# weiquan/salt

Measured on AMD Instinct MI355X. Metric: Mreads/s aligned (100 bp SE, GRCh38+snp144) at 1/2/4/8 MI355X vs CPU ref, higher is better.
Workload: dtype u32; 1 GPU; GRCh38-scale synthetic (SURVEY 8d config 3 = BASELINE configs[2]): 3100000000 bp genome in 24 contigs, 14800000 SNPs, k=21, 1000000 x 100 bp SE reads per GPU per step, 8 distinct resident batches rotated, inputs and results resident in HBM; read_len=100, distinct_batches=8, options=default (-s 50 -m 1000, overlap = k), streams_per_gpu=4

## Files before the change

### salt_amd/csrc/salt_align.hip

```cpp
#include <type_traits>
#include "salt_device.h"
#include "salt_kernels.h"

namespace salt {

#define WSYNC() do { __builtin_amdgcn_fence(__ATOMIC_ACQ_REL, "wavefront"); __builtin_amdgcn_wave_barrier(); \
                     __builtin_amdgcn_fence(__ATOMIC_ACQ_REL, "wavefront"); } while (0)

static constexpr int MAXL = SALT_MAX_READ_LEN;
static constexpr int SLOTS = SALT_MAX_SEED_SLOTS;
static constexpr int MAXLOC = SALT_MAX_LOCATE;
static constexpr int LVK = 31;
static_assert(offsetof(salt_result_t, strand) == 4 && offsetof(salt_result_t, mapq) == 7 && offsetof(salt_result_t, b0) == 8 &&
              offsetof(salt_result_t, b1) == 12 && offsetof(salt_result_t, seq_start) == 16 && offsetof(salt_result_t, seq_end) == 18 &&
              offsetof(salt_result_t, n_hits) == 20 && offsetof(salt_result_t, n_cigar) == 22 && offsetof(salt_result_t, skipped) == 23 &&
              offsetof(salt_result_t, hits) == 24 && sizeof(salt_hit_t) == 8, "salt_result_t header layout");
static constexpr int NHIT = 6;
__device__ __forceinline__ uint32_t mapq_quot(uint32_t x, uint32_t b0)
{
    const uint32_t v = 255u * x;
    return b0 == 1u ? v : b0 == 2u ? v / 2u : b0 == 3u ? v / 3u : v / b0;
}
static constexpr uint32_t INF = 255;

// ... 446 lines not shown
            n_lkt += __shfl_down(n_lkt, o); n_occ_c += __shfl_down(n_occ_c, o); n_occ_r += __shfl_down(n_occ_r, o);
        }
        if (lane_id() == 0) {
            atomicAdd(ctr + SALT_CTR_LKT, n_lkt & 1023u); atomicAdd(ctr + SALT_CTR_OCC_C, n_occ_c); atomicAdd(ctr + SALT_CTR_OCC_R, n_occ_r);
            atomicAdd(ctr + SALT_CTR_D_WLKT, n_lkt & 1023u); atomicAdd(ctr + SALT_CTR_D_COCC_SEED, n_occ_c); atomicAdd(ctr + SALT_CTR_D_ROCC_SEED, n_occ_r);
            atomicAdd(ctr + SALT_CTR_D_SA_SEED, (n_lkt >> 10) & 2047u); atomicAdd(ctr + SALT_CTR_D_TEXT_SEED, n_lkt >> 21);
        }
    }
}

__global__ void __launch_bounds__(256) __attribute__((amdgpu_waves_per_eu(4, 4)))
k_seed_walk(IndexView ix, SeedParams sp, const uint32_t *__restrict__ tb, uint4 *__restrict__ sai_c, uint4 *__restrict__ sai_r,
            const uint4 *__restrict__ wq, const uint32_t *__restrict__ wq_cnt, uint32_t wq_seg_cap, uint32_t r_first, unsigned long long *__restrict__ ctr)
{
    const uint32_t seg = blockIdx.x & (WQ_SEG - 1u);
    const uint32_t wv = (blockIdx.x / WQ_SEG) * 4u + (uint32_t)__builtin_amdgcn_readfirstlane((int)(threadIdx.x >> 6)), nw = (gridDim.x / WQ_SEG) * 4u;
    const uint64_t lt = (1ull << lane_id()) - 1ull;
    const uint32_t la = r_first ? 0u : 1u, lb = la ^ 1u;
    const uint32_t na = wq_cnt[(la * WQ_SEG + seg) * WQ_STRIDE], nb = wq_cnt[(lb * WQ_SEG + seg) * WQ_STRIDE];
    const uint32_t a0 = (uint32_t)((uint64_t)na * wv / nw), a1 = (uint32_t)((uint64_t)na * (wv + 1u) / nw);
    const uint32_t b0 = (uint32_t)((uint64_t)nb * wv / nw), b1 = (uint32_t)((uint64_t)nb * (wv + 1u) / nw);
    const uint4 *qa = wq + (((size_t)la * WQ_SEG + seg) * wq_seg_cap + a0) * WQ_REC, *qb = wq + (((size_t)lb * WQ_SEG + seg) * wq_seg_cap + b0) * WQ_REC;
    const uint32_t tot_a = a1 - a0, tot = tot_a + (b1 - b0);
    const int i_top = (int)((uint32_t)sp.l_seed - ix.r_lkt_len) - 1;
    uint32_t n_aux = 0, n_sa = 0, n_text = 0, n_occ_c = 0, n_occ_r = 0;
    Walk w; w.ph = WK_IDLE; w.k = w.l = w.ext = w.p0 = 0; w.i = 0;
    SeedCtx c = seed_ctx_geom(sp, tb, 0, ix.r_lkt_len);
    uint32_t item = 0, cur = 0;
    bool is_r = false;
    const uint4 *qp = qa;
    for (;;) {
        const uint64_t idle = __ballot(w.ph == WK_IDLE);
        if (cur >= tot && idle == ~0ull) break;
        if (cur < tot) {
            const uint32_t t = cur + (uint32_t)__popcll(idle & lt);
            if (w.ph == WK_IDLE && t < tot) {
                const bool in_a = t < tot_a;
                qp = in_a ? qa + (size_t)t * WQ_REC : qb + (size_t)(t - tot_a) * WQ_REC; is_r = (in_a ? la : lb) == 0u; w.ph = WK_REC;
            }
            const uint32_t nx = cur + (uint32_t)__popcll(idle);
            cur = nx < tot ? nx : tot;
        }
        WalkReq q = walk_req_none();
        if (w.ph == WK_REC) { q.pa = qp; q.na = WQ_REC; }
        else if (w.ph != WK_IDLE) q = is_r ? seed_walk_issue<true>(ix, sp, c, w) : seed_walk_issue<false>(ix, sp, c, w);
        const WalkLoads ld = walk_fetch(q);
        bool done = false;
        uint4 row = make_uint4(1, 0, 0, 0);
        if (w.ph == WK_REC) {
            item = ld.a[0].x;
            c = seed_ctx_geom(sp, tb, item, ix.r_lkt_len);
            c.w0 = ld.a[1].x; c.w1 = ld.a[1].y; c.w2 = ld.a[1].z; c.n0 = ld.a[0].w; c.n1 = ld.a[1].w;
            done = is_r ? seed_walk_begin<true>(sp, c, ld.a[0].y, ld.a[0].z, i_top, w, row) : seed_walk_begin<false>(sp, c, ld.a[0].y, ld.a[0].z, i_top, w, row);
        } else if (w.ph != WK_IDLE) {
            done = is_r ? seed_walk_finish<true>(ix, sp, c, w, ld, row, n_occ_r, n_aux) : seed_walk_finish<false>(ix, sp, c, w, ld, row, n_occ_c, n_aux);
        }
        if (done && row.x <= row.y) { if (is_r) { row.w = sai_r_pack(sp.epoch, row.w); sai_r[item] = row; } else sai_c[item] = row; }
        n_sa += (n_aux >> 10) & 2047u; n_text += n_aux >> 21; n_aux = 0;
    }
    if (ctr) {
        for (int o = 32; o > 0; o >>= 1) { n_sa += __shfl_down(n_sa, o); n_text += __shfl_down(n_text, o); n_occ_c += __shfl_down(n_occ_c, o); n_occ_r += __shfl_down(n_occ_r, o); }
        if (lane_id() == 0) {
            atomicAdd(ctr + SALT_CTR_OCC_C, n_occ_c); atomicAdd(ctr + SALT_CTR_OCC_R, n_occ_r);
            atomicAdd(ctr + SALT_CTR_D_COCC_SEED, n_occ_c); atomicAdd(ctr + SALT_CTR_D_ROCC_SEED, n_occ_r);
            atomicAdd(ctr + SALT_CTR_D_SA_SEED, n_sa); atomicAdd(ctr + SALT_CTR_D_TEXT_SEED, n_text);
        }
    }
}

template <int NS> struct SaiListsT { uint32_t sp[2][NS], ep[2][NS], off[2][NS]; };
struct SaiLists { uint32_t *sp[2], *ep[2], *off[2]; };
template <int NS> __device__ __forceinline__ SaiLists sai_ref(SaiListsT<NS> &a) { return SaiLists{ { a.sp[0], a.sp[1] }, { a.ep[0], a.ep[1] }, { a.off[0], a.off[1] } }; }
struct LvTables { short L[LVK][64]; char A[LVK][64]; };
static constexpr int LLV_K = 12;
static constexpr int LLV_TW = 22;
static constexpr int LLV_N = 64;
static constexpr int LLV_WIN = 4;
static constexpr int LLV_TS = LLV_TW + 2;
static constexpr int LLV_PW = LLV_TW;
static_assert(((8 * (LLV_TW - 1) - LLV_WIN + LLV_K) >> 3) + 2 <= LLV_TS, "text words of the longest window at the widest bound");
static_assert(((8 * (LLV_TW - 1) - LLV_WIN) >> 3) + 2 <= LLV_PW, "pattern words of the longest read");
struct LaneLv { uint32_t T[LLV_TS * LLV_N]; uint32_t P[LLV_PW]; };
struct LvBytes { uint8_t T[MAXL + 4 + 64]; uint8_t P[MAXL + 64]; };
template <int NS, bool LLV>
struct WaveLdsT {
    static constexpr bool HAS_LLV = LLV;
    static constexpr int N_SLOTS = NS;
    uint32_t pm[2][MAXL / 8];
    union U { SaiListsT<NS> sai; typename std::conditional<LLV, LaneLv, uint32_t>::type llv; LvBytes lvb; } u;
    uint8_t  cand_e[MAXLOC];
    uint32_t loci[MAXLOC];
    uint32_t hit_pos[2][NHIT];
    uint8_t  hit_nd[2][NHIT], hit_gap[2][NHIT];
    uint16_t cig[SALT_MAX_CIGAR_OPS];
    int      n_cig;
    alignas(8) uint8_t cargs[128];
};
typedef WaveLdsT<SLOTS, true> WaveLds;
typedef WaveLdsT<32, false> WaveLdsSmall;
typedef WaveLdsT<1, false> WaveLdsCigar;

struct Sai { uint32_t sp, ep, off; };
__device__ __forceinline__ Sai sai_get(const SaiLists &s, int w, int i) { return Sai{ s.sp[w][i], s.ep[w][i], s.off[w][i] }; }
__device__ __forceinline__ void sai_set(SaiLists &s, int w, int i, Sai v) { s.sp[w][i] = v.sp; s.ep[w][i] = v.ep; s.off[w][i] = v.off; }
__device__ __forceinline__ bool sai_ltv(Sai a, Sai b) { return a.ep - a.sp < b.ep - b.sp; }
__device__ __forceinline__ bool sai_lt(const SaiLists &s, int w, int i, int j) { return sai_ltv(sai_get(s, w, i), sai_get(s, w, j)); }
__device__ __forceinline__ void sai_swap(SaiLists &s, int w, int i, int j) { Sai a = sai_get(s, w, i), b = sai_get(s, w, j); sai_set(s, w, i, b); sai_set(s, w, j, a); }

__device__ void sai_insertsort(SaiLists &s, int w, int lo, int hi)
{
    for (int i = lo + 1; i < hi; ++i)
        for (int j = i; j > lo && sai_lt(s, w, j, j - 1); --j) sai_swap(s, w, j, j - 1);
}

__device__ void sai_combsort(SaiLists &s, int w, int base, int n)
{
    const double shrink = 1.2473309501039786540366528676643;
    int gap = n; bool do_swap;
    do {
        if (gap > 2) { gap = (int)(gap / shrink); if (gap == 9 || gap == 10) gap = 11; }
        do_swap = false;
        for (int i = 0; i < n - gap; ++i)
            if (sai_lt(s, w, base + i + gap, base + i)) { sai_swap(s, w, base + i, base + i + gap); do_swap = true; }
    } while (do_swap || gap > 2);
    if (gap != 1) sai_insertsort(s, w, base, base + n);
}

__device__ __attribute__((noinline)) void sai_introsort(SaiLists &s, int w, int n)
{
    if (n < 1) return;
    if (n == 2) { if (sai_lt(s, w, 1, 0)) sai_swap(s, w, 0, 1); return; }
    int d; for (d = 2; (1 << d) < n; ++d) { }
    d <<= 1;
    int st_l[24], st_r[24], st_d[24], top = 0;
    int lo = 0, hi = n - 1;
    for (;;) {
        if (lo < hi) {
            if (--d == 0) { sai_combsort(s, w, lo, hi - lo + 1); hi = lo; continue; }
            int i = lo, j = hi, k = i + ((j - i) >> 1) + 1;
            if (sai_lt(s, w, k, i)) { if (sai_lt(s, w, k, j)) k = j; }
            else k = sai_lt(s, w, j, i) ? i : j;
            Sai rp = sai_get(s, w, k);
            if (k != hi) sai_swap(s, w, k, hi);
            for (;;) {
                do ++i; while (sai_ltv(sai_get(s, w, i), rp));
                do --j; while (i <= j && sai_ltv(rp, sai_get(s, w, j)));
                if (j <= i) break;
                sai_swap(s, w, i, j);
            }
            sai_swap(s, w, i, hi);
            if (i - lo > hi - i) {
                if (i - lo > 16 && top < 24) { st_l[top] = lo; st_r[top] = i - 1; st_d[top] = d; ++top; }
                lo = hi - i > 16 ? i + 1 : hi;
            } else {
                if (hi - i > 16 && top < 24) { st_l[top] = i + 1; st_r[top] = hi; st_d[top] = d; ++top; }
                hi = i - lo > 16 ? i - 1 : lo;
            }
        } else {
            if (top == 0) { sai_insertsort(s, w, 0, n); return; }
            --top; lo = st_l[top]; hi = st_r[top]; d = st_d[top];
        }
    }
}

__device__ void sort_loci(uint32_t *a, uint32_t n)
{
    if (n < 2) return;
    uint32_t P = 2; while (P < n) P <<= 1;
    for (uint32_t i = n + lane_id(); i < P; i += 64) a[i] = 0xFFFFFFFFu;
    WSYNC();
    for (uint32_t k = 2; k <= P; k <<= 1) {
        for (uint32_t j = k >> 1; j > 0; j >>= 1) {
// ... 353 lines not shown
__device__ __forceinline__ void verify_quads_2(const uint32_t *__restrict__ ref, uint32_t ref_len, const uint32_t *pm0, const uint32_t *pm1, uint32_t L,
                                               const uint32_t *c0, uint32_t n0, const uint32_t *c1, uint32_t n1, uint8_t *o0, uint8_t *o1)
{
    constexpr uint32_t CPW = (uint32_t)GW / LN;
    const uint32_t lane = LaneGroup<GW>::lane(), sub = lane & (uint32_t)(LN - 1), q = lane / (uint32_t)LN;
    const uint32_t nw = (L + 7) >> 3, n = n0 + n1;
    const uint32_t nvalid = L > 32u * sub ? (L - 32u * sub < 32u ? L - 32u * sub : 32u) : 0u;
    const bool behind = LN == 8 && GW == 32 && !(4u * sub < nw + 1u);
    uint32_t pa[4], pb[4];
#pragma unroll
    for (int t = 0; t < 4; ++t) { const bool in = (4 * sub + t) < nw; pa[t] = in ? pm0[4 * sub + t] : 0u; pb[t] = in ? pm1[4 * sub + t] : 0u; }
    for (uint32_t b = 0; b < n; b += 4u * CPW) {
        uint32_t pos[4]; u32x4_a4 x[4]; bool act[4], rev[4];
#pragma unroll
        for (int g = 0; g < 4; ++g) {
            if (b + CPW * g >= n) break;
            const uint32_t c = b + CPW * g + q;
            act[g] = c < n; rev[g] = c >= n0;
            pos[g] = act[g] ? (rev[g] ? c1[c - n0] : c0[c]) : 0u;
            if (pos[g] >= ref_len) pos[g] = 0xFFFFFFFFu;
            if (behind) x[g] = u32x4_a4{ 0u, 0u, 0u, 0u };
            else x[g] = *reinterpret_cast<const u32x4_a4 *>(ref + ((pos[g] == 0xFFFFFFFFu ? 0u : pos[g]) >> 3) + 4 * sub);
        }
#pragma unroll
        for (int g = 0; g < 4; ++g) {
            if (b + CPW * g >= n) break;
            const uint32_t pw[4] = { rev[g] ? pb[0] : pa[0], rev[g] ? pb[1] : pa[1], rev[g] ? pb[2] : pa[2], rev[g] ? pb[3] : pa[3] };
            const uint32_t mism = quad_mismatch<LN>(x[g], pos[g], pw, nvalid);
            if (act[g] && sub == 0) {
                const uint32_t c = b + CPW * g + q;
                const uint8_t v = (uint8_t)((mism > 3 || pos[g] == 0xFFFFFFFFu) ? INF : mism);
                if (rev[g]) o1[c - n0] = v; else o0[c] = v;
            }
        }
    }
}

__device__ __attribute__((noinline)) int lv_wave(const uint8_t *T, int tlen, const uint8_t *P, int plen, int k, LvTables *tab, int &d_fin)
{
    const int lane = (int)lane_id();
    const int d = lane - 31;
    const int ad = d < 0 ? -d : d;
    int Lprev = -2;
    const int end0 = plen < tlen ? plen : tlen;
    if (d == 0) { int i = 0; while (i < end0 && (P[i] & T[i]) != 0) ++i; Lprev = i; }
    const int r0 = __shfl(Lprev, 31);
    if (tab) tab->L[0][lane] = (short)Lprev;
    d_fin = 0;
    if (r0 == end0) return plen > end0 ? plen - end0 : 0;
    if (k > LVK - 1) k = LVK - 1;
    for (int e = 1; e <= k; ++e) {
        int left = __shfl_up(Lprev, 1), right = __shfl_down(Lprev, 1);
        if (lane == 0) left = -2;
        if (lane == 63) right = -2;
        const bool active = ad <= e && ad <= LVK - 1;
        int best = Lprev + 1; char act = 'X';
        if (left > best) { best = left; act = 'D'; }
        if (right + 1 > best) { best = right + 1; act = 'I'; }
        int cur = -2;
        if (active) {
            if (P[best] == T[d + best]) {
                int end = plen < tlen - d ? plen : tlen - d;
                if (best >= end) best = end;
                else { int i = best; while (i < end && (P[i] & T[d + i]) != 0) ++i; best = i; }
            }
            cur = best;
        }
        if (tab) { tab->L[e][lane] = (short)cur; tab->A[e][lane] = act; }
        uint64_t reach = __ballot(active && cur == plen);
        if (reach) {
            if (tab) {
                int rank = d == 0 ? 0 : (d < 0 ? 2 * ad - 1 : 2 * ad);
                int my = (active && cur == plen) ? rank : 1000;
                for (int o = 32; o > 0; o >>= 1) { int t = __shfl_xor(my, o); my = t < my ? t : my; }
                d_fin = my == 0 ? 0 : ((my & 1) ? -((my + 1) >> 1) : (my >> 1));
            }
            return e;
        }
        Lprev = cur;
    }
    return -1;
}

__device__ __attribute__((noinline)) uint32_t lv_lanes(LaneLv &s, const uint32_t *pm, int plen, int tlen, int k, bool active)
{
    constexpr int LLV_W = 2 * LLV_K + 1;
    const int lane = (int)lane_id() & (LLV_N - 1);
    const lds_u32 T = as_lds(s.T) + lane, P = as_lds(pm);
    auto fetch = [&](int i, int t, uint32_t &p, uint32_t &x) {
        const lds_u32 pp = P + (i >> 3), tt = T + (t >> 3) * LLV_N;
        const uint32_t p0 = pp[0], p1 = pp[1], t0 = tt[0], t1 = tt[LLV_N];
        p = __funnelshift_r(p0, p1, 4u * (uint32_t)(i & 7));
        x = __funnelshift_r(t0, t1, 4u * (uint32_t)(t & 7));
    };
    auto run_of = [](uint32_t p, uint32_t x) -> int {
        const uint32_t y = p & x;
        const uint32_t z = ~(((y & 0x77777777u) + 0x77777777u) | y) & 0x88888888u;
        return z ? __builtin_ctz(z) >> 2 : 8;
    };
    auto reach = [&](int d, int best, bool gated) -> int {
        uint32_t p, x;
        fetch(best, d + best, p, x);
        const int end = plen < tlen - d ? plen : tlen - d;
        const bool open = !gated || ((p ^ x) & 15u) == 0;
        int run = run_of(p, x), i = best + run;
        if (open && run == 8) while (i < end) { fetch(i, d + i, p, x); run = run_of(p, x); i += run; if (run < 8) break; }
        i = i < end ? i : end;
        return open ? i : best;
    };
    int row[LLV_W];
#pragma unroll
    for (int j = 0; j < LLV_W; ++j) row[j] = -2;
    const int end0 = plen < tlen ? plen : tlen;
    uint32_t result = 255;
    bool done = !active;
    if (active) {
        const int i = reach(0, 0, false);
        row[LLV_K] = i;
        if (i == end0) { result = (uint32_t)(plen > end0 ? plen - end0 : 0); done = true; }
    }
    for (int e = 1; e <= k; ++e) {
        if (__ballot(!done) == 0) break;
        int carry = -2;
#pragma unroll
        for (int d = -LLV_K; d <= LLV_K; ++d) {
            if ((d < 0 ? -d : d) > e) continue;
            const int mid = row[d + LLV_K], right = d < LLV_K ? row[d + LLV_K + 1] : -2;
            int best = mid + 1;
            if (carry > best) best = carry;
            if (right + 1 > best) best = right + 1;
            carry = mid;
            if (!done) {
                best = reach(d, best, true);
                if (best == plen) { result = (uint32_t)e; done = true; }
                else row[d + LLV_K] = best;
            }
        }
    }
    return result;
}

template <int VMAX, bool GAPF>
__device__ __forceinline__ void rule_unsorted(const uint32_t *pos, const uint8_t *val, const uint32_t n, const uint32_t L, const uint32_t ref_len,
                                              uint32_t &bound, bool &any, uint32_t &best_pos, uint32_t &best_v,
                                              uint32_t &n_hits, uint32_t &a0, uint32_t *hit_pos, uint8_t *hit_nd)
{
    const uint32_t lane = lane_id();
    const uint32_t NONE = 0xFFFFFFFFu;
    auto in_range = [&](uint32_t p) -> bool { return GAPF ? !(p + L + 4 >= ref_len) : p < ref_len; };
    uint32_t mp[VMAX + 1];
#pragma unroll
    for (int t = 0; t <= VMAX; ++t) mp[t] = NONE;
    uint32_t my_p = 0, my_v = NONE, n_p = 0;
    for (uint32_t b = 0; b < n; b += 64) {
        const uint32_t i = b + lane;
        uint32_t p = 0, v = NONE;
        if (i < n) { p = pos[i]; v = val[i]; }
        const bool in = i < n && v <= bound && in_range(p);
        if (in) {
#pragma unroll
            for (int t = 0; t <= VMAX; ++t) if (v == (uint32_t)t && p < mp[t]) mp[t] = p;
        }
        uint64_t m = __ballot(in);
        if (m && n_p <= 64u) {
            if (n_p + (uint32_t)__popcll(m) > 64u) n_p = 65u;
            else
                while (m) {
                    const int l = __ffsll((long long)m) - 1;
                    const uint32_t pl = (uint32_t)__builtin_amdgcn_readlane((int)p, l), vl = (uint32_t)__builtin_amdgcn_readlane((int)v, l);
                    if (lane == n_p) { my_p = pl; my_v = vl; }
                    ++n_p; m &= m - 1;
                }
        }
    }
#pragma unroll
    for (int t = 0; t <= VMAX; ++t)
        for (int o = 32; o > 0; o >>= 1) { const uint32_t x = (uint32_t)__shfl_xor((int)mp[t], o); mp[t] = x < mp[t] ? x : mp[t]; }
    uint32_t before[VMAX + 1];
    before[0] = NONE;
#pragma unroll
    for (int t = 1; t <= VMAX; ++t) before[t] = mp[t - 1] < before[t - 1] ? mp[t - 1] : before[t - 1];
    any = false; n_hits = 0;
#pragma unroll
    for (int t = VMAX; t >= 0; --t) if (mp[t] != NONE) { any = true; best_v = (uint32_t)t; best_pos = mp[t]; }
    if (!any) return;
    unsigned long long last = 0;
    const bool in_lanes = n_p <= 64u;
    unsigned long long my_key = ~0ull;
    if (in_lanes && lane < n_p) {
        uint32_t lim = NONE;
#pragma unroll
        for (int t = 1; t <= VMAX; ++t) if (my_v == (uint32_t)t) lim = before[t];
        if (my_p < lim) my_key = ((unsigned long long)my_p << 8) | my_v;
    }
    for (uint32_t h = 0; h < (uint32_t)NHIT; ++h) {
        unsigned long long cur = ~0ull;
        if (in_lanes) { if (h == 0 || my_key > last) cur = my_key; }
        else
        for (uint32_t b = 0; b < n; b += 64) {
            const uint32_t i = b + lane;
            if (i < n) {
                const uint32_t p = pos[i], v = val[i];
                if (v <= bound && in_range(p)) {
                    uint32_t lim = NONE;
#pragma unroll
                    for (int t = 1; t <= VMAX; ++t) if (v == (uint32_t)t) lim = before[t];
                    const unsigned long long key = ((unsigned long long)p << 8) | v;
                    if (p < lim && (h == 0 || key > last) && key < cur) cur = key;
                }
            }
        }
        for (int o = 32; o > 0; o >>= 1) {
            const unsigned long long x = ((unsigned long long)(uint32_t)__shfl_xor((int)(cur >> 32), o) << 32) | (uint32_t)__shfl_xor((int)(uint32_t)cur, o);
            cur = x < cur ? x : cur;
        }
        if (cur == ~0ull) break;
        if (lane == 0) { hit_pos[h] = (uint32_t)(cur >> 8); hit_nd[h] = (uint8_t)(cur & 255u); }
        if (h == 0) a0 = (uint32_t)(cur & 255u);
        last = cur; ++n_hits;
    }
    bound = best_v < bound ? best_v : bound;
}
// ... 10 lines not shown
    auto in_range = [&](uint32_t p) -> bool { return GAPF ? !(p + L + 4 >= ref_len) : p < ref_len; };
    any = false; n_hits = 0;
    if (n == 0) return;
    if (n <= (uint32_t)GW) {
        uint32_t p = 0, v = NONE;
        if (lane < n) { p = pos[lane]; v = val[lane]; }
        const bool ok = v <= bound && in_range(p);
        const mask_t m = G::ballot(ok);
        if (m == 0) return;
        const int l0 = first_bit(m);
        const uint32_t p0 = G::bcast(p, l0);
        if (G::ballot(ok && p != p0) == 0) {
            const uint32_t v0 = G::bcast(v, l0);
            any = true; best_pos = p0; best_v = v0; n_hits = 1; a0 = v0;
            if (lane == 0) { hit_pos[0] = p0; hit_nd[0] = (uint8_t)v0; }
            bound = v0 < bound ? v0 : bound;
            return;
        }
    }
    uint32_t mp[VMAX + 1];
#pragma unroll
    for (int t = 0; t <= VMAX; ++t) mp[t] = NONE;
    for (uint32_t b = 0; b < n; b += GW) {
        const uint32_t i = b + lane;
        uint32_t p = 0, v = NONE;
        if (i < n) { p = pos[i]; v = val[i]; }
        mask_t m = G::ballot(v <= bound && in_range(p));
        while (m) {
            const int l = first_bit(m);
            const uint32_t pl = G::bcast(p, l), vl = G::bcast(v, l);
#pragma unroll
            for (int t = 0; t <= VMAX; ++t) if (vl == (uint32_t)t && pl < mp[t]) mp[t] = pl;
            m &= m - 1;
        }
    }
    uint32_t before[VMAX + 1];
    before[0] = NONE;
#pragma unroll
    for (int t = 1; t <= VMAX; ++t) before[t] = mp[t - 1] < before[t - 1] ? mp[t - 1] : before[t - 1];
#pragma unroll
    for (int t = VMAX; t >= 0; --t) if (mp[t] != NONE) { any = true; best_v = (uint32_t)t; best_pos = mp[t]; }
    if (!any) return;
    uint32_t last_p = 0;
    for (uint32_t h = 0; h < (uint32_t)NHIT; ++h) {
        uint32_t cur_p = NONE, cur_v = 0;
        for (uint32_t b = 0; b < n; b += GW) {
            const uint32_t i = b + lane;
            uint32_t p = 0, v = NONE;
            if (i < n) { p = pos[i]; v = val[i]; }
            uint32_t lim = NONE;
#pragma unroll
            for (int t = 1; t <= VMAX; ++t) if (v == (uint32_t)t) lim = before[t];
            mask_t m = G::ballot(v <= bound && in_range(p) && p < lim && (h == 0 || p > last_p));
            while (m) {
                const int l = first_bit(m);
                const uint32_t pl = G::bcast(p, l);
                if (pl < cur_p) { cur_p = pl; cur_v = G::bcast(v, l); }
                m &= m - 1;
            }
        }
        if (cur_p == NONE) break;
        if (lane == 0) { hit_pos[h] = cur_p; hit_nd[h] = (uint8_t)cur_v; }
        if (h == 0) a0 = cur_v;
        last_p = cur_p; ++n_hits;
    }
    bound = best_v < bound ? best_v : bound;
}

template <class W>
__device__ void lv_unpack(const uint32_t *ref_generic, W &w, int strand, uint32_t L, uint32_t pos)
{
    const gp_u32 ref = as_global(ref_generic);
    const uint32_t tlen = L + 4;
    for (uint32_t i = lane_id(); i < tlen + 48; i += 64) {
        uint32_t p = pos + i;
        w.u.lvb.T[i] = i < tlen ? (uint8_t)((ref[p >> 3] >> (4 * (p & 7u))) & 15u) : (uint8_t)0;
    }
    for (uint32_t i = lane_id(); i < L + 48; i += 64) {
        w.u.lvb.P[i] = i < L ? (uint8_t)((w.pm[strand][i >> 3] >> (4 * (i & 7u))) & 15u) : (uint8_t)0;
    }
    WSYNC();
}

template <class W>
__device__ __attribute__((noinline)) void lv_cigar(const uint32_t *ref, W &w, LvTables *tabp, int strand, uint32_t L, uint32_t pos, int k)
{
    LvTables &tab = *tabp;
    lv_unpack(ref, w, strand, L, pos);
    int d_fin = 0;
    WSYNC();
    int e = lv_wave(w.u.lvb.T, (int)L + 4, w.u.lvb.P, (int)L, k, &tab, d_fin);
    __threadfence_block();
    WSYNC();
    if (lane_id() == 0) {
        int n = 0;
        uint16_t *cg = w.cig;
        if (e == 0) { cg[n++] = (uint16_t)((L << 4) | 0u); }
        else if (e > 0) {
            char act[LVK + 1]; int matched[LVK + 1];
            int cd = d_fin;
            for (int ce = e; ce >= 1; --ce) {
                char a = tab.A[ce][cd + 31];
                act[ce] = a;
                int cur = tab.L[ce][cd + 31];
                if (a == 'I') { matched[ce] = cur - tab.L[ce - 1][cd + 1 + 31] - 1; cd += 1; }
                else if (a == 'D') { matched[ce] = cur - tab.L[ce - 1][cd - 1 + 31]; cd -= 1; }
                else { matched[ce] = cur - tab.L[ce - 1][cd + 31] - 1; }
            }
            int acc = tab.L[0][31];
            int ce = 1;
            while (ce <= e) {
                char a = act[ce]; int cnt = 1;
                while (ce + 1 <= e && matched[ce] == 0 && act[ce + 1] == a) { ++cnt; ++ce; }
                if (a == 'X') acc += cnt;
                else {
                    if (acc != 0 && n < SALT_MAX_CIGAR_OPS) { cg[n++] = (uint16_t)((acc << 4) | 0); }
                    acc = 0;
                    if (n < SALT_MAX_CIGAR_OPS) cg[n++] = (uint16_t)((cnt << 4) | (a == 'I' ? 1 : 2));
                }
                if (matched[ce] > 0) acc += matched[ce];
                ++ce;
            }
            if (acc != 0 && n < SALT_MAX_CIGAR_OPS) cg[n++] = (uint16_t)((acc << 4) | 0);
        }
        w.n_cig = n;
    }
    WSYNC();
}

__device__ __forceinline__ void lane_text(const uint32_t *__restrict__ ref, uint32_t *T, uint32_t pos, uint32_t tl)
{
    const uint32_t w0 = pos >> 3, sh = (pos & 7u) * 4u, nwt = (tl + 7) >> 3, nst = ((tl - LLV_WIN + LLV_K) >> 3) + 2;
    uint32_t wv[LLV_TW + 1];
#pragma unroll
    for (int j = 0; j <= LLV_TW; ++j) wv[j] = (uint32_t)j <= nwt ? ref[w0 + (uint32_t)j] : 0u;
#pragma unroll
    for (int j = 0; j < LLV_TW; ++j) {
        uint32_t word = 0;
        if ((uint32_t)j < nwt) {
            word = __funnelshift_r(wv[j], wv[j + 1], sh);
            const uint32_t rem = tl - (uint32_t)j * 8;
            if (rem < 8) word &= (1u << (4 * rem)) - 1u;
        }
        if ((uint32_t)j < nst) T[j * LLV_N] = word;
    }
#pragma unroll
    for (int j = LLV_TW; j < LLV_TS; ++j) if ((uint32_t)j < nst) T[j * LLV_N] = 0u;
}
template <class F>
__device__ __forceinline__ void lane_pattern(uint32_t *P, uint32_t nw, uint32_t first, uint32_t step, F word)
{
    for (uint32_t j = first; j < (uint32_t)LLV_PW; j += step) P[j] = j < nw ? word(j) : 0u;
}

__device__ __forceinline__ uint32_t store_gap_list(const uint32_t *loci, uint32_t n, uint32_t L, uint32_t ref_len, uint32_t *__restrict__ dst)
{
    const uint32_t lane = lane_id();
    const uint64_t lt = (1ull << lane) - 1ull;
    uint32_t n_out = 0;
    for (uint32_t b = 0; b < n; b += 64) {
        const uint32_t i = b + lane;
        const uint32_t pos = i < n ? loci[i] : 0u;
        const bool keep = i < n && !(pos + L + 4 >= ref_len);
        const uint64_t m = __ballot(keep);
        if (keep) dst[n_out + (uint32_t)__popcll(m & lt)] = pos;
        n_out += (uint32_t)__popcll(m);
    }
    return n_out;
}

template <bool PE, bool GL, class W>
__device__ __forceinline__ void align_general(const IndexView ix, const AlignParams ap, W &w, const uint32_t r,
                              const uint32_t *__restrict__ pm,
                              const uint4 *__restrict__ sai_c, const uint4 *__restrict__ sai_r,
                              salt_result_t *__restrict__ results, unsigned long long *__restrict__ ctr,
                              unsigned long long *phase, LvTables *lvtab, const GapBufs g, uint32_t *pe_loci, uint8_t *pe_cand)
{
    const uint32_t lane = lane_id();
    const uint64_t lt = (1ull << lane) - 1ull;
    const uint32_t *rec = pm + (uint64_t)r * ap.pg.pm_stride;
    const uint32_t L = rec[2 * ap.pg.nw8];
    salt_result_t *out = results + r;
    uint32_t c_sa_c = 0, c_sa_r = 0, c_verify = 0, c_vwords = 0, c_lv = 0, c_loci = 0, c_ctx_rej = 0, c_ctx_rows = 0;
    PhaseClock pc(phase);
    const uint64_t rt0 = phase ? __builtin_amdgcn_s_memrealtime() : 0;
    constexpr bool glob = GL;
    uint32_t *loci = glob ? pe_loci : w.loci;
    uint8_t *cand_e = glob ? pe_cand : w.cand_e;
    const uint32_t loci_cap = PE ? PE_LOCI_CAP : (uint32_t)MAXLOC;

    const uint32_t nw = (L + 7) >> 3;
    uint32_t n_amb = 0;
    for (uint32_t t = lane; t < 2 * nw; t += 64) {
        const uint32_t s = t >= nw, j = s ? t - nw : t;
        const uint32_t word = rec[s * ap.pg.nw8 + j];
        w.pm[s][j] = word;
        if (!s) n_amb += (uint32_t)__popc(word & (word >> 1) & (word >> 2) & (word >> 3) & 0x11111111u);
    }
    if (ap.max_amb < L) { for (int o = 32; o > 0; o >>= 1) n_amb += (uint32_t)__shfl_xor((int)n_amb, o); }
    else n_amb = 0;
    WSYNC();
    uint32_t q_pos = 0xFFFFFFFFu; uint32_t q_strand = 3, q_ndiff = 255, q_gap = 255;
    const bool too_short = L < (uint32_t)ap.l_seed;
    if (n_amb > ap.max_amb) {
        if (lane == 0) {
            out->pos = q_pos; out->strand = 3; out->n_diff = 255; out->is_gap = 255; out->mapq = 0;
            out->b0 = -1; out->b1 = -1; out->seq_start = 0; out->seq_end = (uint16_t)(L - 1);
            out->n_hits[0] = out->n_hits[1] = 0; out->n_cigar = 0; out->skipped = 1;
        }
        return;
    }
    pc.stamp(SALT_CTR_T_LOAD);
    uint32_t bound = 3;
    bool found[2] = { false, false };
    uint32_t n_hits_s[2] = { 0, 0 };
    uint32_t a0[2] = { 0, 0 };
    uint32_t n_cand_nogap = 0, n_loc_s[2] = { 0, 0 };
    if (!too_short)
    for (int strand = 0; strand < 2; ++strand) {
        pc.stamp(SALT_CTR_T_SCAN);
        const CandStats cs = build_candidates_call<PE, GL>(CandArgs{ ix.c_sa, ix.r_pos, sai_c, sai_r, ix.ref_len, ap.spr, ap.max_locate, r, L, strand, false, phase, pe_loci, loci_cap, ap.pe, false, ap.epoch, ix.r_ctx, ix.c_ctx, ix.ctx_k }, w);
        if (glob) { loci = cs.in_lds ? w.loci : pe_loci; cand_e = cs.in_lds ? w.cand_e : pe_cand; }
        pc.t = phase ? __builtin_amdgcn_s_memtime() : 0;
        const uint32_t n_loc = cs.n_cand; c_sa_c += cs.n_sa_c; c_sa_r += cs.n_sa_r; c_loci += cs.n_loci; c_ctx_rej += cs.n_ctx_rej; c_ctx_rows += cs.n_ctx_rows;
        uint32_t call_best_n = INF, call_best_pos = 0;
        if (SALT_DIAG_VAL(ap.heavy_stop) == 1) continue;
        auto verify_all = [&](uint32_t n) {
            if (L <= 120) verify_quads<8>(ix.ref, ix.ref_len, w.pm[strand], L, loci, n, cand_e);
            else if (L <= 248) verify_two_phase(ix.ref, ix.ref_len, w.pm[strand], L, loci, n, cand_e);
            else for (uint32_t i = lane; i < n; i += 64) cand_e[i] = (uint8_t)mismatch_capped(ix, w.pm[strand], L, loci[i]);
            WSYNC();
        };
        verify_all(n_loc);
        pc.stamp(SALT_CTR_T_VERIFY);
        if (SALT_DIAG_VAL(ap.heavy_stop) == 2) continue;
// ... 340 lines not shown
        uint32_t n_hits_s[2] = { 0, 0 }, a0[2] = { 0, 0 };
        for (int strand = 0; strand < 2; ++strand) {
            const uint32_t n = g.gn[2 * slot + strand];
            const size_t row = g.goff[2 * slot + strand];
            bool any = false; uint32_t bp = 0, bv = 0;
            rule_unsorted<LLV_K, true>(g.gloci + row, g.ge + row, n, L, ix.ref_len, bound, any, bp, bv, n_hits_s[strand], a0[strand],
                                       w.hit_pos[strand], w.hit_nd[strand]);
            if (any) { q_pos = bp; q_ndiff = bv; q_gap = 1; q_strand = (uint32_t)strand; }
        }
        WSYNC();
        int b0 = (int)q_ndiff, b1 = 100000, tot = 0;
        uint32_t nh[2] = { 0, 0 };
        uint32_t sel_idx[2][SALT_MAX_HITS];
        for (int s = 0; s < 2 && tot < ap.max_hits; ++s)
            for (uint32_t j = 0; j < n_hits_s[s]; ++j) {
                const uint32_t p = w.hit_pos[s][j];
                if (p == 0xFFFFFFFFu || p == q_pos) continue;
                if (a0[s] <= q_ndiff) {
                    if ((int)a0[s] <= b1) b1 = (int)a0[s];
                    if (nh[s] < SALT_MAX_HITS) sel_idx[s][nh[s]] = j;
                    ++nh[s]; ++tot;
                }
                if (tot == ap.max_hits) break;
            }
        uint32_t mapq = 0;
        if (b0 != 0) {
            const uint32_t x = (uint32_t)(b0 > b1 ? b0 - b1 : b1 - b0);
            const uint64_t q = mapq_quot(x, (uint32_t)b0);
            mapq = q < 254 ? (uint32_t)q : 254u;
        }
        const uint32_t n_cig_items = q_pos != 0xFFFFFFFFu ? 1u + nh[0] + nh[1] : 0u;
        const uint32_t first_cig = ap.pe ? 1u : 0u;
        if (lane == 0) {
            out->pos = q_pos; out->strand = (uint8_t)q_strand; out->n_diff = (uint8_t)q_ndiff; out->is_gap = (uint8_t)q_gap;
            out->mapq = (uint8_t)mapq; out->b0 = b0; out->b1 = b1; out->seq_start = 0; out->seq_end = (uint16_t)(L - 1);
            out->n_hits[0] = (uint8_t)nh[0]; out->n_hits[1] = (uint8_t)nh[1]; out->skipped = 0; out->n_cigar = 0;
            for (int s = 0; s < 2; ++s)
                for (uint32_t j = 0; j < nh[s]; ++j) {
                    const uint32_t h = sel_idx[s][j];
                    out->hits[s][j].pos = w.hit_pos[s][h]; out->hits[s][j].n_diff = w.hit_nd[s][h];
                    out->hits[s][j].is_gap = 1; out->hits[s][j].strand = (uint16_t)s;
                }
            if (n_cig_items > first_cig) {
                const uint32_t base = atomicAdd(&g.gctl->cigar_items, n_cig_items - first_cig);
                for (uint32_t c = first_cig; c < n_cig_items; ++c) g.cq[base + c - first_cig] = (r << 3) | c;
            }
            if (ctr) atomicMax(ctr + SALT_CTR_MAX_GAPFIN, ((unsigned long long)(__builtin_amdgcn_s_memrealtime() - rt0) << 32) | r);
        }
        WSYNC();
    }
}

__global__ void __launch_bounds__(64)
k_cigar(IndexView ix, PackGeom pg, const uint32_t *__restrict__ pm, salt_result_t *__restrict__ results,
        const uint32_t *__restrict__ items, const uint32_t *__restrict__ count, uint32_t *__restrict__ head, uint32_t cap_items,
        LvTables *__restrict__ lvtab)
{
    __shared__ WaveLdsCigar w;
    __shared__ uint32_t s_item;
    const uint32_t lane = lane_id();
    const uint32_t n_items = *count < cap_items ? *count : cap_items;
    struct { PackGeom pg; } ap = { pg };
    bool first = true;
    for (;;) {
        if (threadIdx.x == 0) s_item = first ? blockIdx.x : sw_pull(head, 1u, gridDim.x, n_items);
        first = false;
        WSYNC();
        const uint32_t it = s_item;
        WSYNC();
        if (it >= n_items) break;
        const uint32_t item = items[it], which = item & 7u, r = item >> 3;
        salt_result_t *out = results + r;
        const uint32_t *rec = pm + (uint64_t)r * ap.pg.pm_stride;
        const uint32_t L = rec[2 * ap.pg.nw8];
        uint32_t strand, pos, k;
        if (which == 0) { strand = out->strand; pos = out->pos; k = out->n_diff; }
        else {
            const uint32_t h = which - 1, n0 = out->n_hits[0];
            strand = h >= n0; const uint32_t j = strand ? h - n0 : h;
            pos = out->hits[strand][j].pos; k = out->hits[strand][j].n_diff;
        }
        for (uint32_t t = lane; t < (L + 7) >> 3; t += 64) w.pm[strand][t] = rec[strand * ap.pg.nw8 + t];
        WSYNC();
        lv_cigar(ix.ref, w, lvtab + blockIdx.x, (int)strand, L, pos, (int)k);
        uint16_t *dst = which == 0 ? out->cigar : out->hit_cigar[which - 1];
        if (lane < (uint32_t)w.n_cig) dst[lane] = w.cig[lane];
        if (lane == 0) { if (which == 0) out->n_cigar = (uint8_t)w.n_cig; else out->hit_n_cigar[which - 1] = (uint8_t)w.n_cig; }
        WSYNC();
    }
}

__host__ __device__ __forceinline__ uint32_t qseg_cap(uint32_t n_reads) { return n_reads / QUEUE_RANGES + 8u; }
__device__ __forceinline__ void queue_push(uint32_t *__restrict__ qseg, QueueRange *__restrict__ ranges, uint32_t n_reads, uint32_t r)
{
    const uint32_t s = (r >> 2) & (QUEUE_RANGES - 1u);
    qseg[(size_t)s * qseg_cap(n_reads) + atomicAdd(&ranges[s].push, 1u)] = r;
}
__device__ __forceinline__ uint32_t *retry_segs(uint32_t *qseg, uint32_t n_reads) { return qseg + (size_t)QUEUE_RANGES * qseg_cap(n_reads); }
__device__ __forceinline__ void retry_push(uint32_t *__restrict__ qseg, QueueRange *__restrict__ ranges, uint32_t n_reads, uint32_t r)
{
    const uint32_t s = (r >> 2) & (QUEUE_RANGES - 1u);
    retry_segs(qseg, n_reads)[(size_t)s * qseg_cap(n_reads) + atomicAdd(&ranges[s].retry, 1u)] = r;
}
__global__ void __launch_bounds__(256)
k_queue_pack(const uint32_t *__restrict__ qseg, const QueueRange *__restrict__ ranges, uint32_t n_reads, uint32_t *__restrict__ queue, SeCtl *__restrict__ ctl)
{
    __shared__ uint32_t base_s, cnt_s;
    if (threadIdx.x == 0) {
        uint32_t base = 0, total = 0;
        for (uint32_t s = 0; s < QUEUE_RANGES; ++s) { const uint32_t c = ranges[s].push; if (s < blockIdx.x) base += c; total += c; }
        base_s = base; cnt_s = ranges[blockIdx.x].push;
        if (blockIdx.x == 0) ctl->light_queued = total;
    }
    __syncthreads();
    const uint32_t *src = qseg + (size_t)blockIdx.x * qseg_cap(n_reads);
    for (uint32_t i = threadIdx.x; i < cnt_s; i += 256) queue[base_s + i] = src[i];
}

static constexpr int LT_LOCI = 128;
static constexpr int LT_MAXL = 160;
static constexpr int L2_SLOTS = 8;
static constexpr int L4_SLOTS = 4;
#ifndef SALT_L4_ROWS
#define SALT_L4_ROWS 16
#endif
static constexpr int L4_ROWS = SALT_L4_ROWS;

template <int SLOTS, int PMW, int LOCI> struct LightRec {
    uint32_t pm[2][PMW];
    uint32_t sp[4][SLOTS], off[4][SLOTS];
    uint32_t pre[4][SLOTS + 1];
    uint32_t loci[2][LOCI];
    uint32_t hit_pos[2][NHIT];
    uint8_t  hit_nd[2][NHIT];
    uint8_t  val[2][LOCI];
};
template <int GW> using LightLds = LightRec<GW / 4, GW == 64 ? LT_MAXL / 8 : GW == 32 ? 32 : 16, GW == 16 ? 2 * L4_ROWS : LT_LOCI>;
static_assert(sizeof(LightLds<32>) == 1996 && 8 * sizeof(LightLds<16>) <= 4 * sizeof(LightLds<32>), "eight quarter records in the LDS of four half-wave ones");

template <int GW, int LN, bool INSTR>
__device__ __forceinline__ void light_read(const IndexView &ix, const AlignParams &ap, const uint32_t *__restrict__ pm,
                                           const uint4 *__restrict__ sai_c, const uint4 *__restrict__ sai_r, salt_result_t *__restrict__ results,
                                           uint32_t *__restrict__ queue , QueueRange *__restrict__ ranges,
                                           unsigned long long *__restrict__ ctr, LightLds<GW> &w, const uint32_t r)
{
    typedef LaneGroup<GW> G;
    typedef typename G::mask_t mask_t;
    constexpr uint32_t SLOTS = GW / 4, HALF = GW / 2;
    constexpr uint32_t LMAX = LN == 4 ? 120u : LN == 8 ? 248u : (uint32_t)LT_MAXL;
    static_assert(LMAX <= 8 * sizeof(w.pm[0]) / 4 && (LN != 0 || LMAX <= 248u), "the read fits the record and the window check");
    const uint32_t lane = G::lane();
    const mask_t lt = G::below();
    const uint32_t *rec = pm + (uint64_t)r * ap.pg.pm_stride;
    const uint32_t L = rec[2 * ap.pg.nw8];
    bool heavy = L > LMAX || L < (uint32_t)ap.l_seed || ap.spr > SLOTS || ap.max_locate < 2 * 64;
    uint32_t c_sa_c = 0, c_sa_r = 0, c_verify = 0, c_loci = 0;
    const bool prof = INSTR && ctr && (r & 127u) == 0;
    uint64_t tp = prof ? __builtin_amdgcn_s_memtime() : 0;
    auto stamp = [&](int slot) {
        if (!prof) return;
        const uint64_t n = __builtin_amdgcn_s_memtime();
        if (lane == 0) atomicAdd(ctr + slot, (unsigned long long)(n - tp));
        tp = n;
    };
    auto locate = [&](uint32_t l, uint32_t j, uint32_t of, uint32_t &p) -> bool {
        p = ((of >> 31) ? j : (l & 1) ? ix.r_pos[j] : ix.c_sa[j]) - (of & 0x7FFFFFFFu);
        return (l & 1) ? !(p > ix.ref_len || p + L > ix.ref_len) : !(p + L > ix.ref_len);
// ... 627 lines not shown
```

Baseline: 556.9 Mreads/s.

## Trace CIGAR Landau-Vishkin in LDS with packed nibble text instead of global tables

Adds a fast CIGAR path for small edit distances and short reads. It loads packed 4-bit text and pattern words into LDS and runs a wave-wide Landau-Vishkin trace (one diagonal per lane) that stores the L/A tables as bytes in LDS. This replaces the byte-unpacked text and the per-block global LvTables that the backtrace used to read. The nibble-compare helpers are refactored into a shared struct, and the traceback now reads from whichever table was filled. The cigar kernel call is inlined. Reads with larger edit distances fall back to the old path. Risks: the union overlays and the byte-sized L entries must not overflow.

```diff
diff --git a/salt_amd/csrc/salt_align.hip b/salt_amd/csrc/salt_align.hip
--- a/salt_amd/csrc/salt_align.hip
+++ b/salt_amd/csrc/salt_align.hip
@@ -552,12 +552,15 @@
 static_assert(((8 * (LLV_TW - 1) - LLV_WIN) >> 3) + 2 <= LLV_PW, "pattern words of the longest read");
 struct LaneLv { uint32_t T[LLV_TS * LLV_N]; uint32_t P[LLV_PW]; };
 struct LvBytes { uint8_t T[MAXL + 4 + 64]; uint8_t P[MAXL + 64]; };
+struct LvTrace { uint32_t T[LLV_TS], P[LLV_PW]; uint8_t L[LLV_K + 1][2 * LLV_K + 2], A[LLV_K + 1][2 * LLV_K + 2]; };
+struct LvWalk { uint16_t matched[LVK + 1]; uint8_t act[LVK + 1]; };
+static_assert(sizeof(LvTrace) <= sizeof(LvBytes) && sizeof(LvWalk) <= offsetof(LvTrace, L), "inside the byte strings; the walk clear of lv_trace's tables");
 template <int NS, bool LLV>
 struct WaveLdsT {
     static constexpr bool HAS_LLV = LLV;
     static constexpr int N_SLOTS = NS;
     uint32_t pm[2][MAXL / 8];
-    union U { SaiListsT<NS> sai; typename std::conditional<LLV, LaneLv, uint32_t>::type llv; LvBytes lvb; } u;
+    union U { SaiListsT<NS> sai; typename std::conditional<LLV, LaneLv, uint32_t>::type llv; LvBytes lvb; LvTrace lvt; LvWalk walk; } u;
     uint8_t  cand_e[MAXLOC];
     uint32_t loci[MAXLOC];
     uint32_t hit_pos[2][NHIT];
@@ -1077,23 +1080,25 @@
     return -1;
 }
 
-__device__ __attribute__((noinline)) uint32_t lv_lanes(LaneLv &s, const uint32_t *pm, int plen, int tlen, int k, bool active)
-{
-    constexpr int LLV_W = 2 * LLV_K + 1;
-    const int lane = (int)lane_id() & (LLV_N - 1);
-    const lds_u32 T = as_lds(s.T) + lane, P = as_lds(pm);
-    auto fetch = [&](int i, int t, uint32_t &p, uint32_t &x) {
-        const lds_u32 pp = P + (i >> 3), tt = T + (t >> 3) * LLV_N;
-        const uint32_t p0 = pp[0], p1 = pp[1], t0 = tt[0], t1 = tt[LLV_N];
+template <int TS>
+struct LvNib {
+    lds_u32 T, P;
+    int plen, tlen;
+    __device__ __forceinline__ void fetch(int i, int t, uint32_t &p, uint32_t &x) const
+    {
+        const lds_u32 pp = P + (i >> 3), tt = T + (t >> 3) * TS;
+        const uint32_t p0 = pp[0], p1 = pp[1], t0 = tt[0], t1 = tt[TS];
         p = __funnelshift_r(p0, p1, 4u * (uint32_t)(i & 7));
         x = __funnelshift_r(t0, t1, 4u * (uint32_t)(t & 7));
-    };
-    auto run_of = [](uint32_t p, uint32_t x) -> int {
+    }
+    __device__ __forceinline__ static int run_of(uint32_t p, uint32_t x)
+    {
         const uint32_t y = p & x;
         const uint32_t z = ~(((y & 0x77777777u) + 0x77777777u) | y) & 0x88888888u;
         return z ? __builtin_ctz(z) >> 2 : 8;
-    };
-    auto reach = [&](int d, int best, bool gated) -> int {
+    }
+    __device__ __forceinline__ int reach(int d, int best, bool gated) const
+    {
         uint32_t p, x;
         fetch(best, d + best, p, x);
         const int end = plen < tlen - d ? plen : tlen - d;
@@ -1102,7 +1107,14 @@
         if (open && run == 8) while (i < end) { fetch(i, d + i, p, x); run = run_of(p, x); i += run; if (run < 8) break; }
         i = i < end ? i : end;
         return open ? i : best;
-    };
+    }
+};
+
+__device__ __attribute__((noinline)) uint32_t lv_lanes(LaneLv &s, const uint32_t *pm, int plen, int tlen, int k, bool active)
+{
+    constexpr int LLV_W = 2 * LLV_K + 1;
+    const int lane = (int)lane_id() & (LLV_N - 1);
+    const LvNib<LLV_N> op = { as_lds(s.T) + lane, as_lds(pm), plen, tlen };
     int row[LLV_W];
 #pragma unroll
     for (int j = 0; j < LLV_W; ++j) row[j] = -2;
@@ -1110,7 +1122,7 @@
     uint32_t result = 255;
     bool done = !active;
     if (active) {
-        const int i = reach(0, 0, false);
+        const int i = op.reach(0, 0, false);
         row[LLV_K] = i;
         if (i == end0) { result = (uint32_t)(plen > end0 ? plen - end0 : 0); done = true; }
     }
@@ -1126,13 +1138,47 @@
             if (right + 1 > best) best = right + 1;
             carry = mid;
             if (!done) {
-                best = reach(d, best, true);
+                best = op.reach(d, best, true);
                 if (best == plen) { result = (uint32_t)e; done = true; }
                 else row[d + LLV_K] = best;
             }
         }
     }
     return result;
+}
+
+__device__ __forceinline__ int lv_trace(LvTrace &s, int plen, int tlen, int k, int &d_fin)
+{
+    const int lane = (int)lane_id(), d = lane - 31, ad = d < 0 ? -d : d;
+    const LvNib<1> op = { as_lds(s.T), as_lds(s.P), plen, tlen };
+    const bool mine = ad <= LLV_K;
+    const int col = mine ? d + LLV_K : 0;
+    const int end0 = plen < tlen ? plen : tlen;
+    const int r0 = op.reach(0, 0, false);
+    int Lprev = d == 0 ? r0 : -2;
+    if (mine) s.L[0][col] = (uint8_t)(Lprev + 2);
+    d_fin = 0;
+    if (r0 == end0) return plen > end0 ? plen - end0 : 0;
+    if (k > LLV_K) k = LLV_K;
+    for (int e = 1; e <= k; ++e) {
+        const int left = __shfl_up(Lprev, 1), right = __shfl_down(Lprev, 1);
+        const bool active = ad <= e;
+        int best = Lprev + 1; uint8_t act = 'X';
+        if (left > best) { best = left; act = 'D'; }
+        if (right + 1 > best) { best = right + 1; act = 'I'; }
+        int cur = -2;
+        if (active) cur = op.reach(d, best, true);
+        if (mine) { s.L[e][col] = (uint8_t)(cur + 2); s.A[e][col] = act; }
+        if (__ballot(active && cur == plen)) {
+            const int rank = d == 0 ? 0 : (d < 0 ? 2 * ad - 1 : 2 * ad);
+            int my = (active && cur == plen) ? rank : 1000;
+            for (int o = 32; o > 0; o >>= 1) { const int t = __shfl_xor(my, o); my = t < my ? t : my; }
+            d_fin = my == 0 ? 0 : ((my & 1) ? -((my + 1) >> 1) : (my >> 1));
+            return e;
+        }
+        Lprev = cur;
+    }
+    return -1;
 }
 
 template <int VMAX, bool GAPF>
@@ -1309,36 +1355,87 @@
     WSYNC();
 }
 
+__device__ __forceinline__ void lane_text(const uint32_t *__restrict__ ref, uint32_t *T, uint32_t pos, uint32_t tl)
+{
+    const uint32_t w0 = pos >> 3, sh = (pos & 7u) * 4u, nwt = (tl + 7) >> 3, nst = ((tl - LLV_WIN + LLV_K) >> 3) + 2;
+    uint32_t wv[LLV_TW + 1];
+#pragma unroll
+    for (int j = 0; j <= LLV_TW; ++j) wv[j] = (uint32_t)j <= nwt ? ref[w0 + (uint32_t)j] : 0u;
+#pragma unroll
+    for (int j = 0; j < LLV_TW; ++j) {
+        uint32_t word = 0;
+        if ((uint32_t)j < nwt) {
+            word = __funnelshift_r(wv[j], wv[j + 1], sh);
+            const uint32_t rem = tl - (uint32_t)j * 8;
+            if (rem < 8) word &= (1u << (4 * rem)) - 1u;
+        }
+        if ((uint32_t)j < nst) T[j * LLV_N] = word;
+    }
+#pragma unroll
+    for (int j = LLV_TW; j < LLV_TS; ++j) if ((uint32_t)j < nst) T[j * LLV_N] = 0u;
+}
+template <class F>
+__device__ __forceinline__ void lane_pattern(uint32_t *P, uint32_t nw, uint32_t first, uint32_t step, F word)
+{
+    for (uint32_t j = first; j < (uint32_t)LLV_PW; j += step) P[j] = j < nw ? word(j) : 0u;
+}
+
+__device__ __forceinline__ void wave_text(const uint32_t *__restrict__ ref, uint32_t *T, uint32_t pos, uint32_t tl)
+{
+    const uint32_t j = lane_id(), w0 = pos >> 3, sh = (pos & 7u) * 4u, nwt = (tl + 7) >> 3, nst = ((tl - LLV_WIN + LLV_K) >> 3) + 2;
+    const uint32_t wv = w0 + j <= (pos + tl - 1) >> 3 ? ref[w0 + j] : 0u;
+    const uint32_t nx = (uint32_t)__shfl_down((int)wv, 1);
+    uint32_t word = 0;
+    if (j < nwt) {
+        word = __funnelshift_r(wv, nx, sh);
+        const uint32_t rem = tl - j * 8;
+        if (rem < 8) word &= (1u << (4 * rem)) - 1u;
+    }
+    if (j < nst) T[j] = word;
+}
+
 template <class W>
-__device__ __attribute__((noinline)) void lv_cigar(const uint32_t *ref, W &w, LvTables *tabp, int strand, uint32_t L, uint32_t pos, int k)
+__device__ __forceinline__ void lv_cigar_here(const uint32_t *ref, W &w, LvTables *tabp, int strand, uint32_t L, uint32_t pos, int k)
 {
     LvTables &tab = *tabp;
-    lv_unpack(ref, w, strand, L, pos);
-    int d_fin = 0;
-    WSYNC();
-    int e = lv_wave(w.u.lvb.T, (int)L + 4, w.u.lvb.P, (int)L, k, &tab, d_fin);
-    __threadfence_block();
+    const bool in_lds = k <= LLV_K && L + 4 <= 8u * (LLV_TW - 1);
+    int d_fin = 0, e;
+    if (in_lds) {
+        lane_pattern(w.u.lvt.P, (L + 7) >> 3, lane_id(), 64u, [&](uint32_t j) { return w.pm[strand][j]; });
+        wave_text(ref, w.u.lvt.T, pos, L + 4);
+        WSYNC();
+        e = lv_trace(w.u.lvt, (int)L, (int)L + 4, k, d_fin);
+    } else {
+        lv_unpack(ref, w, strand, L, pos);
+        WSYNC();
+        e = lv_wave(w.u.lvb.T, (int)L + 4, w.u.lvb.P, (int)L, k, &tab, w.n_cig);
+        __threadfence_block();
+        WSYNC();
+        d_fin = w.n_cig;
+    }
     WSYNC();
     if (lane_id() == 0) {
+        auto Lat = [&](int ee, int d) -> int { return in_lds ? (int)w.u.lvt.L[ee][d + LLV_K] - 2 : (int)tab.L[ee][d + 31]; };
+        auto Aat = [&](int ee, int d) -> char { return in_lds ? (char)w.u.lvt.A[ee][d + LLV_K] : tab.A[ee][d + 31]; };
         int n = 0;
         uint16_t *cg = w.cig;
         if (e == 0) { cg[n++] = (uint16_t)((L << 4) | 0u); }
         else if (e > 0) {
-            char act[LVK + 1]; int matched[LVK + 1];
+            uint8_t *act = w.u.walk.act; uint16_t *matched = w.u.walk.matched;
             int cd = d_fin;
             for (int ce = e; ce >= 1; --ce) {
-                char a = tab.A[ce][cd + 31];
-                act[ce] = a;
-                int cur = tab.L[ce][cd + 31];
-                if (a == 'I') { matched[ce] = cur - tab.L[ce - 1][cd + 1 + 31] - 1; cd += 1; }
-                else if (a == 'D') { matched[ce] = cur - tab.L[ce - 1][cd - 1 + 31]; cd -= 1; }
-                else { matched[ce] = cur - tab.L[ce - 1][cd + 31] - 1; }
-            }
-            int acc = tab.L[0][31];
+                char a = Aat(ce, cd);
+                act[ce] = (uint8_t)a;
+                int cur = Lat(ce, cd);
+                if (a == 'I') { matched[ce] = (uint16_t)(cur - Lat(ce - 1, cd + 1) - 1); cd += 1; }
+                else if (a == 'D') { matched[ce] = (uint16_t)(cur - Lat(ce - 1, cd - 1)); cd -= 1; }
+                else { matched[ce] = (uint16_t)(cur - Lat(ce - 1, cd) - 1); }
+            }
+            int acc = Lat(0, 0);
             int ce = 1;
             while (ce <= e) {
-                char a = act[ce]; int cnt = 1;
-                while (ce + 1 <= e && matched[ce] == 0 && act[ce + 1] == a) { ++cnt; ++ce; }
+                char a = (char)act[ce]; int cnt = 1;
+                while (ce + 1 <= e && matched[ce] == 0 && act[ce + 1] == (uint8_t)a) { ++cnt; ++ce; }
                 if (a == 'X') acc += cnt;
                 else {
                     if (acc != 0 && n < SALT_MAX_CIGAR_OPS) { cg[n++] = (uint16_t)((acc << 4) | 0); }
@@ -1354,30 +1451,10 @@
     }
     WSYNC();
 }
-
-__device__ __forceinline__ void lane_text(const uint32_t *__restrict__ ref, uint32_t *T, uint32_t pos, uint32_t tl)
-{
-    const uint32_t w0 = pos >> 3, sh = (pos & 7u) * 4u, nwt = (tl + 7) >> 3, nst = ((tl - LLV_WIN + LLV_K) >> 3) + 2;
-    uint32_t wv[LLV_TW + 1];
-#pragma unroll
-    for (int j = 0; j <= LLV_TW; ++j) wv[j] = (uint32_t)j <= nwt ? ref[w0 + (uint32_t)j] : 0u;
-#pragma unroll
-    for (int j = 0; j < LLV_TW; ++j) {
-        uint32_t word = 0;
-        if ((uint32_t)j < nwt) {
-            word = __funnelshift_r(wv[j], wv[j + 1], sh);
-            const uint32_t rem = tl - (uint32_t)j * 8;
-            if (rem < 8) word &= (1u << (4 * rem)) - 1u;
-        }
-        if ((uint32_t)j < nst) T[j * LLV_N] = word;
-    }
-#pragma unroll
-    for (int j = LLV_TW; j < LLV_TS; ++j) if ((uint32_t)j < nst) T[j * LLV_N] = 0u;
-}
-template <class F>
-__device__ __forceinline__ void lane_pattern(uint32_t *P, uint32_t nw, uint32_t first, uint32_t step, F word)
-{
-    for (uint32_t j = first; j < (uint32_t)LLV_PW; j += step) P[j] = j < nw ? word(j) : 0u;
+template <class W>
+__device__ __attribute__((noinline)) void lv_cigar(const uint32_t *ref, W &w, LvTables *tabp, int strand, uint32_t L, uint32_t pos, int k)
+{
+    lv_cigar_here(ref, w, tabp, strand, L, pos, k);
 }
 
 __device__ __forceinline__ uint32_t store_gap_list(const uint32_t *loci, uint32_t n, uint32_t L, uint32_t ref_len, uint32_t *__restrict__ dst)
@@ -1884,7 +1961,7 @@
         }
         for (uint32_t t = lane; t < (L + 7) >> 3; t += 64) w.pm[strand][t] = rec[strand * ap.pg.nw8 + t];
         WSYNC();
-        lv_cigar(ix.ref, w, lvtab + blockIdx.x, (int)strand, L, pos, (int)k);
+        lv_cigar_here(ix.ref, w, lvtab + blockIdx.x, (int)strand, L, pos, (int)k);
         uint16_t *dst = which == 0 ? out->cigar : out->hit_cigar[which - 1];
         if (lane < (uint32_t)w.n_cig) dst[lane] = w.cig[lane];
         if (lane == 0) { if (which == 0) out->n_cigar = (uint8_t)w.n_cig; else out->hit_n_cigar[which - 1] = (uint8_t)w.n_cig; }
```

Result: no change. 555.1 Mreads/s (-0.3%).
